# MITIBMxGraph/SALIENT_plusplus

Hardware: AMD Instinct MI355X
Metric: sampled_edges_per_sec (higher is better)
Workload: dtype int64/fp16-copy

## Files before the change

### include/spp.h

```cpp
#ifndef SPP_H
#define SPP_H

#include <stddef.h>
#include <stdint.h>

#ifdef __cplusplus
extern "C" {
#endif

#define SPP_ABI_VERSION 6
#define SPP_MAX_HOPS 8
#define SPP_MAX_PARTS 64

typedef int spp_status;
enum {
  SPP_OK = 0,
  SPP_ERR_INVALID = -1,
  SPP_ERR_HIP = -2,
  SPP_ERR_CAPACITY = -3,
  SPP_ERR_STATE = -4
};

int spp_abi_version(void);
const char* spp_last_error(void);
// ... 37 lines not shown
  int64_t cache_map_len;
} spp_partition_cfg;

typedef struct spp_sampler_opts {
  int32_t col32;
  int32_t deg_tags;
  int32_t row_stubs;
  int32_t rng_arena;
  int64_t rng_arena_mb;
  int32_t fuse_scatter;
  int32_t flag_tiled;
  int32_t rows_coalesced;
  int32_t dedup_preread;
  int64_t fuse_max_edges;
  int64_t initial_edge_cap;
  int64_t reserved[4];
} spp_sampler_opts;

typedef struct spp_sampler_cfg {
  const int64_t* rowptr_dev;
  const int64_t* col_dev;
  int64_t num_nodes;
  int64_t nnz;
  int32_t num_hops;
  int64_t sizes[SPP_MAX_HOPS];
  int64_t max_batch;
  int32_t num_slots;
  int32_t device;
  int32_t replace;
  spp_partition_cfg part;
  int64_t graph_generation;
// ... 5 lines not shown
  int32_t deg_tags;
  int32_t row_stubs;
  int32_t rng_arena;
  int32_t idbits, tag_cap;
  int32_t num_hops;
  int32_t dedup_buckets_log2;
  int32_t dedup_table_slots;
  int32_t generic[SPP_MAX_HOPS];
  int32_t fused_pick[SPP_MAX_HOPS];
  int32_t flag_tiled[SPP_MAX_HOPS];
  int32_t rows_coalesced[SPP_MAX_HOPS];
  int32_t bucket_log2[SPP_MAX_HOPS];
  double col32_ms, row_stubs_ms, rng_arena_ms;
  int64_t col32_bytes, row_stubs_bytes, rng_arena_bytes;
  int64_t rng_arena_batches;
} spp_sampler_info;

typedef struct spp_mfg_counts {
  int64_t num_nodes;
  int64_t num_seeds;
  int32_t num_hops;
  int64_t T[SPP_MAX_HOPS];
  int64_t S[SPP_MAX_HOPS];
  int64_t E[SPP_MAX_HOPS];
  int64_t draws;
  int64_t part_counts[SPP_MAX_PARTS + 2];
} spp_mfg_counts;

typedef struct spp_mfg_out {
  int64_t* n_id;
// ... 846 lines not shown
```

### salient_plusplus_amd/_native.py

```python
import ctypes as C
import os

_HERE = os.path.dirname(os.path.abspath(__file__))
LIB_PATH = os.path.join(_HERE, "libspp_hip.so")

SPP_MAX_HOPS = 8
SPP_MAX_PARTS = 64

p = C.c_void_p
i32 = C.c_int32
i64 = C.c_int64
u32 = C.c_uint32


class PartitionCfg(C.Structure):
    _fields_ = [("num_parts", i32), ("rank", i32), ("offsets", i64 * (SPP_MAX_PARTS + 1)),
                ("use_cache", i32), ("cache_map_dev", p), ("cache_map_len", i64)]


class SamplerOpts(C.Structure):
    _fields_ = [("col32", i32), ("deg_tags", i32), ("row_stubs", i32), ("rng_arena", i32), ("rng_arena_mb", i64),
                ("fuse_scatter", i32), ("flag_tiled", i32), ("rows_coalesced", i32), ("dedup_preread", i32),
                ("fuse_max_edges", i64), ("initial_edge_cap", i64), ("reserved", i64 * 4)]


class SamplerCfg(C.Structure):
    _fields_ = [("rowptr_dev", p), ("col_dev", p), ("num_nodes", i64), ("nnz", i64),
                ("num_hops", i32), ("sizes", i64 * SPP_MAX_HOPS), ("max_batch", i64),
                ("num_slots", i32), ("device", i32), ("replace", i32), ("part", PartitionCfg),
                ("graph_generation", i64), ("opts", SamplerOpts)]


class SamplerInfo(C.Structure):
    _fields_ = [("col32", i32), ("deg_tags", i32), ("row_stubs", i32), ("rng_arena", i32), ("idbits", i32),
                ("tag_cap", i32), ("num_hops", i32), ("dedup_buckets_log2", i32), ("dedup_table_slots", i32),
                ("generic", i32 * SPP_MAX_HOPS), ("fused_pick", i32 * SPP_MAX_HOPS), ("flag_tiled", i32 * SPP_MAX_HOPS),
                ("rows_coalesced", i32 * SPP_MAX_HOPS), ("bucket_log2", i32 * SPP_MAX_HOPS),
                ("col32_ms", C.c_double), ("row_stubs_ms", C.c_double), ("rng_arena_ms", C.c_double),
                ("col32_bytes", i64), ("row_stubs_bytes", i64), ("rng_arena_bytes", i64), ("rng_arena_batches", i64)]


class MfgCounts(C.Structure):
    _fields_ = [("num_nodes", i64), ("num_seeds", i64), ("num_hops", i32),
                ("T", i64 * SPP_MAX_HOPS), ("S", i64 * SPP_MAX_HOPS), ("E", i64 * SPP_MAX_HOPS),
                ("draws", i64), ("part_counts", i64 * (SPP_MAX_PARTS + 2))]


class MfgOut(C.Structure):
    _fields_ = [("n_id", p), ("rowptr", p * SPP_MAX_HOPS), ("col", p * SPP_MAX_HOPS),
                ("parts", p), ("cached", p), ("perm", p), ("row_addr", p), ("x_remote", p)]


SPP_ELEM_F32, SPP_ELEM_F16, SPP_ELEM_BF16 = 0, 1, 2
SPP_BN_ACT_NONE, SPP_BN_ACT_RELU, SPP_BN_ACT_LEAKY_RELU = 0, 1, 2
# ... 383 lines not shown
```

### salient_plusplus_amd/csrc/sampler.hip

```cpp
#include "spp_internal.h"

#include <hipcub/hipcub.hpp>

#include <algorithm>
#include <chrono>
#include <cstdlib>
#include <cstring>
#include <vector>

#include <map>
#include <memory>
#include <mutex>
#include <tuple>

#include "fp8_body.hip.h"
#include "gather_body.hip.h"
#include "partition_common.hip.h"

#ifndef SPP_TILE_NT
#define SPP_TILE_NT 1024
#endif
#include "mt19937.hip.h"
#include "sampler_internal.h"

// ... 1984 lines not shown
  void* cub_tmp = nullptr;
  size_t cub_tmp_bytes = 0;
};

struct ResolvedOpts {
  int col32 = 1;
  int deg_tags = 1;
  int row_stubs = -1;
  int rng_arena = -1;
  int64_t rng_arena_words = 0;
  int fuse = 1;
  int64_t fuse_max_edges = 262144;
  bool flag_tiled = true, rows_coalesced = true, dedup_preread = false;
};

struct HopPlan {
  bool self_prefix = false;
  bool fused = false;
  bool flag_tiled = false;
  bool rows_coal = false;
  unsigned row_lds = 0;
  unsigned lds_fused = 0;
  int64_t tile_cap = 0;
};

struct spp_sampler {
  spp_sampler_cfg cfg{};
  ResolvedOpts opt{};
  HopPlan plan[SPP_MAX_HOPS];
  int rng_arena_decision = -1;
  double col32_ms = 0, stubs_ms = 0;
  hipEvent_t arena_t0 = nullptr, arena_t1 = nullptr;
  double rng_arena_ms = 0;
  bool arena_timed = false;
  int64_t tcap[SPP_MAX_HOPS + 1];
  int64_t ecap[SPP_MAX_HOPS];
  int64_t dcap = 0;
  bool generic[SPP_MAX_HOPS];
  bool any_generic = false;
  DedupGeom geom{};
  int cb_log2[SPP_MAX_HOPS];
  int lds_log2 = 12;
  int64_t bytes = 0;
  std::vector<SlotHost> slots;
// ... 61 lines not shown
  SPP_REQUIRE(cfg->max_batch > 0 && cfg->num_slots > 0, "spp_sampler_create: max_batch and num_slots must be > 0");
  const spp_partition_cfg& pc = cfg->part;
  SPP_REQUIRE(pc.num_parts >= 0 && pc.num_parts <= SPP_MAX_PARTS, "spp_sampler_create: num_parts %d not in [0,%d]",
              pc.num_parts, SPP_MAX_PARTS);
  if (pc.num_parts > 0) {
    SPP_REQUIRE(pc.rank >= 0 && pc.rank < pc.num_parts, "spp_sampler_create: rank %d out of [0,%d)", pc.rank,
                pc.num_parts);
    SPP_REQUIRE(!pc.use_cache || (pc.cache_map_dev && pc.cache_map_len > 0),
                "spp_sampler_create: use_cache without a cache map");
    for (int m = 0; m < pc.num_parts; ++m)
      SPP_REQUIRE(pc.offsets[m] <= pc.offsets[m + 1], "spp_sampler_create: partition offsets must be non-decreasing");
    SPP_REQUIRE(pc.offsets[0] <= 0 && pc.offsets[pc.num_parts] >= cfg->num_nodes,
                "spp_sampler_create: partition offsets [%lld,%lld) do not cover the %lld nodes",
                (long long)pc.offsets[0], (long long)pc.offsets[pc.num_parts], (long long)cfg->num_nodes);
  }
  int ndev = spp_device_count();
  SPP_REQUIRE(ndev > 0, "spp_sampler_create: no HIP device available (the on-GPU sampler has no CPU fallback)");
  SPP_HIP_TRY(hipSetDevice(cfg->device));

  auto* s = new spp_sampler();
  s->cfg = *cfg;
  if (const char* e = getenv("SPP_XCD_AFFINITY")) s->xcd_affinity = atoi(e) != 0;
  {
    const spp_sampler_opts& o = cfg->opts;
    auto env_int = [](const char* name, long long dflt) -> long long {
      const char* e = getenv(name);
      return e && *e ? atoll(e) : dflt;
    };
    auto sw = [&](int32_t field, const char* name, int dflt) -> int {
      if (field) return field > 0 ? 1 : 0;
// ... 6 lines not shown
    else {
      const long long m = env_int("SPP_ROW_STUBS", -1);
      r.row_stubs = m < 0 ? -1 : (m > 0 ? 1 : 0);
    }
    const bool env_budget = getenv("SPP_RNG_ARENA_MB") != nullptr;
    const long long mb = o.rng_arena_mb > 0 ? o.rng_arena_mb : env_int("SPP_RNG_ARENA_MB", 16384);
    r.rng_arena_words = (mb < 0 ? 0 : mb) * (int64_t)(1 << 20) / 4;
    if (o.rng_arena) r.rng_arena = o.rng_arena > 0 ? 1 : 0;
    else r.rng_arena = (o.rng_arena_mb > 0 || env_budget) ? 1 : -1;
    if (o.fuse_scatter) r.fuse = o.fuse_scatter < 0 ? 0 : std::min(o.fuse_scatter, 2);
    else r.fuse = (int)std::max<long long>(0, std::min<long long>(2, env_int("SPP_FUSE_SCATTER", 1)));
    r.fuse_max_edges = o.fuse_max_edges > 0 ? o.fuse_max_edges : env_int("SPP_FUSE_MAX_EDGES", 262144);
    r.flag_tiled = sw(o.flag_tiled, "SPP_FLAG_TILED", 1) != 0;
    r.rows_coalesced = sw(o.rows_coalesced, "SPP_ROWS_COALESCED", 1) != 0;
    r.dedup_preread = sw(o.dedup_preread, "SPP_DEDUP_PREREAD", 0) != 0;
  }
  const int H = cfg->num_hops;
  const int64_t node_bound = cfg->num_nodes + cfg->max_batch;
  s->tcap[0] = cfg->max_batch;
  int64_t etmp = 1;
  for (int h = 0; h < H; ++h) {
    const int64_t f = cfg->sizes[h];
    s->generic[h] = (f < 0 || f > kFastMaxFanout);
    s->any_generic |= s->generic[h];
    if (f >= 0) {
      s->ecap[h] = s->tcap[h] * f;
      s->tcap[h + 1] = std::min(s->tcap[h] * (1 + f), node_bound);
      s->dcap += f * s->tcap[h];
    } else {
      s->ecap[h] = cfg->opts.initial_edge_cap > 0 ? cfg->opts.initial_edge_cap
// ... 18 lines not shown
  s->geom.nb_log2 = nb_log2;
  s->geom.nb = 1 << nb_log2;
  const int64_t per_bucket = (ucap + s->geom.nb - 1) / s->geom.nb;
  s->geom.kcap = (int32_t)std::min<int64_t>(per_bucket + per_bucket / 2 + 256, 0x7fffffff);
  s->lds_log2 = per_bucket > 6144 ? 14 : (per_bucket > 1536 ? 13 : (per_bucket > 820 ? 12 : 11));
  for (int h = 0; h < H; ++h) {
    int c = std::max(0, nb_log2 - kMaxFineLog2);
    while (c < nb_log2 && (s->tcap[h + 1] >> c) > bucket_nodes) ++c;
    s->cb_log2[h] = c;
  }
  const int nb = s->geom.nb;
  int64_t tmax = 0;
  for (int h = 0; h < H; ++h) tmax = std::max(tmax, s->tcap[h]);
  const int64_t nblk_max = std::max(ceil_div(tmax, kNT), ceil_div(etmp, kNT)) + 1;
  const int nslots = cfg->num_slots;
  if (pc.num_parts > 0) {
    s->part.P = pc.num_parts;
    s->part.rank = pc.rank;
    s->part.use_cache = pc.use_cache ? 1 : 0;
    s->part.cache_map = pc.cache_map_dev;
    s->part.cache_len = pc.cache_map_len;
    s->part.off.n = pc.num_parts + 1;
    for (int m = 0; m <= pc.num_parts; ++m) s->part.off.v[m] = pc.offsets[m];
    s->part.nblk_cap = (int32_t)ceil_div(ucap, kNT);
  }

  s->slots.resize(nslots);
  spp_status rc = SPP_OK;
  void* v = nullptr;
  rc = dev_alloc(s, &v, sizeof(SlotPtrs) * (size_t)nslots);
// ... 43 lines not shown
      A(p.parts, int32_t, ucap);
      A(p.pcached, int32_t, ucap);
      A(p.pperm, int32_t, ucap);
      A(p.psrc, int2, ucap);
      A(p.pbucket, uint8_t, ucap);
      A(p.pblk, int32_t, (int64_t)(s->part.P + 1) * s->part.nblk_cap);
    }
#undef A
    p.kcount = s->counts + (size_t)i * (size_t)s->counts_per_slot;
    p.bfill = p.kcount + nb;
    p.ctr = p.bfill + nb;
    p.ovfc = p.ctr + 1;
    p.st = s->d_states + i;
    sl.host_state = s->h_states + i;
    if (rc == SPP_OK) {
      sl.etmp_cap = etmp;
      hipError_t e = hipMalloc((void**)&p.cval, sizeof(int32_t) * (size_t)etmp);
      const size_t n_bucketed = (size_t)(region_for(etmp) + etmp);
      if (e == hipSuccess) e = hipMalloc((void**)&p.bpairs, sizeof(unsigned long long) * n_bucketed);
      if (e == hipSuccess) e = hipMalloc((void**)&p.evals, sizeof(uint32_t) * (size_t)etmp);
      if (e == hipSuccess) e = hipMalloc((void**)&p.inv, sizeof(uint32_t) * (size_t)etmp);
      if (e == hipSuccess) e = hipMalloc((void**)&p.tidx, sizeof(uint16_t) * (size_t)etmp);
      if (e == hipSuccess) e = hipMalloc((void**)&p.res, sizeof(uint32_t) * n_bucketed);
      if (e == hipSuccess) e = hipMalloc((void**)&p.fwords, rank_bytes(etmp));
      if (e == hipSuccess) p.fsum = reinterpret_cast<int32_t*>(reinterpret_cast<char*>(p.fwords) + rank_off_fsum(etmp));
      if (e != hipSuccess) {
        set_error("spp_sampler_create: hipMalloc of edge scratch failed: %s", hipGetErrorString(e));
        rc = SPP_ERR_HIP;
      }
      s->bytes += 14 * etmp + 12 * (int64_t)n_bucketed + (int64_t)rank_bytes(etmp);
    }
    if (rc == SPP_OK && (hipEventCreateWithFlags(&sl.done, hipEventDisableTiming) != hipSuccess ||
                         hipEventCreateWithFlags(&sl.exported, hipEventDisableTiming) != hipSuccess)) {
      set_error("spp_sampler_create: hipEventCreate failed");
      rc = SPP_ERR_HIP;
    }
  }
  if (rc == SPP_OK && cfg->nnz > 0 && s->opt.col32) {
    std::lock_guard<std::mutex> lk(g_col32_mu);
    int idbits = 1;
    while (idbits < 32 && ((int64_t)1 << idbits) < cfg->num_nodes) ++idbits;
    const bool want_tags = s->opt.deg_tags && idbits <= 29;
    const auto key = std::make_tuple((const void*)cfg->col_dev, cfg->nnz, (int)cfg->device, cfg->graph_generation,
                                     want_tags ? 1 : 0);
    std::shared_ptr<Col32> c = g_col32[key].lock();
// ... 168 lines not shown
  s->workers[1].reset();
  (void)hipSetDevice(s->cfg.device);
  (void)hipDeviceSynchronize();
  for (auto& sl : s->slots) {
    if (sl.done) (void)hipEventDestroy(sl.done);
    if (sl.exported) (void)hipEventDestroy(sl.exported);
    if (sl.p.cval) (void)hipFree(sl.p.cval);
    if (sl.p.bpairs) (void)hipFree(sl.p.bpairs);
    if (sl.p.evals) (void)hipFree(sl.p.evals);
    if (sl.p.inv) (void)hipFree(sl.p.inv);
    if (sl.p.tidx) (void)hipFree(sl.p.tidx);
    if (sl.p.res) (void)hipFree(sl.p.res);
    if (sl.p.fwords) (void)hipFree(sl.p.fwords);
    if (sl.cub_tmp) (void)hipFree(sl.cub_tmp);
  }
  if (s->rng_arena) (void)hipFree(s->rng_arena);
  if (s->rng_arena_seeds_dev) (void)hipFree(s->rng_arena_seeds_dev);
  if (s->rng_arena_ready) (void)hipEventDestroy(s->rng_arena_ready);
  if (s->arena_t0) (void)hipEventDestroy(s->arena_t0);
  if (s->arena_t1) (void)hipEventDestroy(s->arena_t1);
  if (s->inputs_ready) (void)hipEventDestroy(s->inputs_ready);
  if (s->cache_bits_ready) (void)hipEventDestroy(s->cache_bits_ready);
  if (s->cache_bits) (void)hipFree(s->cache_bits);
  if (s->h_states) (void)hipHostFree(s->h_states);
  if (s->deliver_stream) (void)hipStreamDestroy(s->deliver_stream);
  for (auto st : s->work_streams)
    if (st) (void)hipStreamDestroy(st);
  if (s->comm_stream) (void)hipStreamDestroy(s->comm_stream);
  for (auto& d : s->dargs_host)
    if (d) (void)hipHostFree(d);
// ... 46 lines not shown
  if (s->arena_timed) {
    (void)hipSetDevice(s->cfg.device);
    float ms = 0.f;
    if (hipEventSynchronize(s->arena_t1) == hipSuccess && hipEventElapsedTime(&ms, s->arena_t0, s->arena_t1) == hipSuccess)
      s->rng_arena_ms = ms;
    (void)hipGetLastError();
    s->arena_timed = false;
  }
  out->col32_ms = s->col32_ms;
  out->row_stubs_ms = s->stubs_ms;
  out->rng_arena_ms = s->rng_arena_ms;
  out->col32_bytes = s->col32 ? (int64_t)sizeof(int32_t) * (s->cfg.nnz + 16) : 0;
  out->row_stubs_bytes = s->stubs ? (int64_t)sizeof(int32_t) * kStubInts * s->cfg.num_nodes : 0;
  out->rng_arena_bytes = 4 * s->rng_arena_words;
  out->rng_arena_batches = (int64_t)s->rng_arena_seeds.size();
  return SPP_OK;
}

static spp_status grow_edge_scratch(spp_sampler* s, int slot, int h, int64_t need, hipStream_t st) {
  SlotHost& sl = s->slots[(size_t)slot];
  bool changed = false;
  if (need > sl.etmp_cap) {
    int64_t cap = std::max(need, sl.etmp_cap * 2);
    RankWord* old_fwords = sl.p.fwords;
    int32_t* old_fsum = sl.p.fsum;
    const int64_t old_cap = sl.etmp_cap;
    (void)hipFree(sl.p.cval); (void)hipFree(sl.p.bpairs); (void)hipFree(sl.p.evals);
    (void)hipFree(sl.p.inv); (void)hipFree(sl.p.res); (void)hipFree(sl.p.tidx);
    sl.p.tidx = nullptr;
    sl.p.cval = nullptr; sl.p.bpairs = nullptr; sl.p.evals = nullptr; sl.p.fwords = nullptr;
// ... 17 lines not shown
  }
  if (need > sl.ecap_dyn[h]) {
    int64_t cap = std::max(need, sl.ecap_dyn[h] * 2);
    void* v = nullptr;
    SPP_HIP_TRY(hipMalloc(&v, sizeof(int32_t) * (size_t)cap));
    s->allocs.push_back(v);
    sl.p.out_col[h] = static_cast<int32_t*>(v);
    s->bytes += 4 * cap;
    sl.ecap_dyn[h] = cap;
    changed = true;
  }
  if (changed) SPP_TRY(upload_slot(s, slot, st));
  return SPP_OK;
}

namespace spp {

int sampler_max_group(const spp_sampler* s) { return s->any_generic ? 1 : kMaxGroup; }

hipStream_t sampler_work_stream(spp_sampler* s, int i) {
  static const int n_streams = [] {
    const char* e = getenv("SPP_WORK_STREAMS");
    const int v = e ? atoi(e) : 2;
    return v < 1 ? 1 : (v > kMaxWorkStreams ? kMaxWorkStreams : v);
  }();
  hipStream_t& st = s->work_streams[i % n_streams];
  if (!st && create_data_stream(&st, true) != hipSuccess) st = nullptr;
  return st;
}

// ... 105 lines not shown
  SlotHost& lead = s->slots[(size_t)first_slot];
  const int32_t interleave = s->xcd_affinity ? 1 : 0;
  auto GG = [&](unsigned gx) { return GroupGrid{(int32_t)first_slot, (int32_t)n, gx, interleave}; };

  static const struct Dup { int count, pick, flag, rows; } dup = [] {
    Dup d{1, 1, 1, 1};
    if (const char* e = getenv("SPP_WHATIF_DUP")) {
      if (strstr(e, "count")) d.count = 2;
      if (strstr(e, "pick")) d.pick = 2;
      if (strstr(e, "flag")) d.flag = 2;
      if (strstr(e, "rows")) d.rows = 2;
    }
    return d;
  }();
  const DedupGeom geom = s->geom;
  const int prof = prof_begin(SPP_PROF_CHAIN, st, n);
  SPP_HIP_TRY(hipMemsetAsync(lead.p.kcount, 0, sizeof(int32_t) * (size_t)s->counts_per_slot * (size_t)n, st));
  const unsigned gseed = (unsigned)ceil_div(max_seeds, kNT);
  ga.grid = GG(gseed);
  hipLaunchKernelGGL(k_seed_init, dim3(gseed * gy), dim3(kNT), 0, st, s->d_slots, ga, geom, rowptr, stubs,
                     (int32_t)s->cfg.sizes[0], replace, s->tag_cap);
  const uint32_t idmask = s->idmask;
  const uint32_t pick_mask = s->use_tags ? 0xffffffffu : idmask;
  const int32_t row_idbits = s->use_tags ? s->idbits : 32;
  for (int h = 0; h < H; ++h) {
    const int32_t f = (int32_t)s->cfg.sizes[h];
    const unsigned gt = (unsigned)std::max<int64_t>(1, ceil_div(s->tcap[h], kNT));
    const HopPlan& pl = s->plan[h];
    const unsigned row_lds = pl.row_lds;
    for (int rep = 0; h > 0 && rep < dup.count; ++rep) {
      const unsigned gc = (gt + kNT / kWave - 1) / (kNT / kWave);
      hipLaunchKernelGGL(k_hop_count, dim3((gc) * gy), dim3(kNT), 0, st, s->d_slots, GG(gc), rowptr, stubs, s->use_tags ? 1 : 0, h, f, replace, (int32_t)s->tcap[h]);
    }
    const int32_t ecap_dev =
        s->generic[h] ? 0x7fffffff : (int32_t)std::min<int64_t>(lead.ecap_dyn[h], 0x7fffffff);
    const int32_t self_prefix = pl.self_prefix ? 1 : 0;
    if (!self_prefix)
      hipLaunchKernelGGL(k_hop_scan, dim3((1) * gy), dim3(kScanNT), 0, st, s->d_slots, GG(1), h, f, ecap_dev, s->dcap);
    const FuseArgs fa_plain{};
    unsigned ge;
    for (int rep = 0; !s->generic[h] && rep < dup.pick - 1; ++rep)
      if (col32 && stubs && s->use_tags)
        hipLaunchKernelGGL((k_hop_pick<false, int32_t, true, true>), dim3((gt) * gy), dim3(kNT), row_lds, st, s->d_slots, GG(gt),
                           col32, stubs, h, f, replace, self_prefix, ecap_dev, s->dcap, (int32_t)s->tcap[h], pick_mask, fa_plain);
    const int32_t cb = s->cb_log2[h];
    const unsigned nbk = 1u << cb;
    const int64_t pcap = std::max<int64_t>(1, s->generic[h] ? 0 : s->ecap[h]);
    const bool fused = pl.fused;
    const int64_t tile_cap = pl.tile_cap;
    const unsigned lds_fused = pl.lds_fused;
    if (!s->generic[h]) {
      if (fused) {
        FuseArgs fa{cb, bucket_cap(pcap, nbk), (int32_t)region_for(lead.etmp_cap), idmask, (int32_t)(row_lds / sizeof(int32_t)), (int32_t)tile_cap};
        const unsigned lds = lds_fused;
        hipLaunchKernelGGL((k_hop_pick<false, int32_t, true, true, true>), dim3((gt) * gy), dim3(kNT), lds, st, s->d_slots, GG(gt),
                           col32, stubs, h, f, replace, self_prefix, ecap_dev, s->dcap, (int32_t)s->tcap[h], pick_mask, fa);
      } else if (col32 && stubs && s->use_tags)
        hipLaunchKernelGGL((k_hop_pick<false, int32_t, true, true>), dim3((gt) * gy), dim3(kNT), row_lds, st, s->d_slots, GG(gt),
                           col32, stubs, h, f, replace, self_prefix, ecap_dev, s->dcap, (int32_t)s->tcap[h], pick_mask, fa_plain);
      else if (col32 && stubs)
        hipLaunchKernelGGL((k_hop_pick<false, int32_t, true>), dim3((gt) * gy), dim3(kNT), row_lds, st, s->d_slots, GG(gt),
                           col32, stubs, h, f, replace, self_prefix, ecap_dev, s->dcap, (int32_t)s->tcap[h], pick_mask, fa_plain);
      else if (col32)
        hipLaunchKernelGGL((k_hop_pick<false, int32_t, false>), dim3((gt) * gy), dim3(kNT), row_lds, st, s->d_slots, GG(gt),
                           col32, stubs, h, f, replace, self_prefix, ecap_dev, s->dcap, (int32_t)s->tcap[h], pick_mask, fa_plain);
      else if (stubs)
        hipLaunchKernelGGL((k_hop_pick<false, int64_t, true>), dim3((gt) * gy), dim3(kNT), row_lds, st, s->d_slots, GG(gt),
                           col, stubs, h, f, replace, self_prefix, ecap_dev, s->dcap, (int32_t)s->tcap[h], pick_mask, fa_plain);
      else
        hipLaunchKernelGGL((k_hop_pick<false, int64_t, false>), dim3((gt) * gy), dim3(kNT), row_lds, st, s->d_slots, GG(gt),
                           col, stubs, h, f, replace, self_prefix, ecap_dev, s->dcap, (int32_t)s->tcap[h], pick_mask, fa_plain);
      ge = (unsigned)std::max<int64_t>(1, ceil_div(s->ecap[h], kNT));
    } else {
      SPP_HIP_TRY(hipMemcpyAsync(lead.host_state, lead.p.st, sizeof(SlotState), hipMemcpyDeviceToHost, st));
      SPP_HIP_TRY(hipStreamSynchronize(st));
      const int64_t E = lead.host_state->E[h];
      if (lead.host_state->error) break;
      SPP_TRY(grow_edge_scratch(s, first_slot, h, E, st));
      ge = (unsigned)std::max<int64_t>(1, ceil_div(E, kNT));
      hipLaunchKernelGGL((k_hop_pick<true, int64_t, false>), dim3((gt) * gy), dim3(kNT), sizeof(int32_t) * kNT, st, s->d_slots,
                         GG(gt), col, stubs, h, f, replace, 0, ecap_dev, s->dcap, (int32_t)s->tcap[h], pick_mask, fa_plain);
      if (col32)
        hipLaunchKernelGGL(k_hop_expand_generic<int32_t>, dim3((ge) * gy), dim3(kNT), 0, st, s->d_slots, GG(ge), col32,
                           h, f, replace, idmask);
      else
        hipLaunchKernelGGL(k_hop_expand_generic<int64_t>, dim3((ge) * gy), dim3(kNT), 0, st, s->d_slots, GG(ge), col,
                           h, f, replace, idmask);
    }
    const int32_t region = (int32_t)region_for(lead.etmp_cap);
    const bool dedup_preread = s->opt.dedup_preread;
    const int32_t last = ((h == H - 1) ? 1 : 0) | (!dedup_preread ? 2 : 0);
    const int32_t hop_word = h | (s->cb_log2[h] << 8) | (last << 16);
    const int64_t pcap_h = s->generic[h] ? std::max<int64_t>(1, lead.host_state->E[h]) : pcap;
    const unsigned gsc = (unsigned)std::max<int64_t>(1, ceil_div((int64_t)ge * kNT, kScatterTile));
    const unsigned sc_lds = (unsigned)(sizeof(int32_t) * 2 * nbk + (sizeof(uint32_t) + sizeof(uint16_t)) * kScatterTile);
    const int32_t bcap = bucket_cap(pcap_h, nbk);
    const bool flag_tiled = pl.flag_tiled;
    if (!fused)
      hipLaunchKernelGGL(k_bucket_scatter, dim3((gsc) * gy), dim3(kTileNT), sc_lds, st, s->d_slots, GG(gsc), h, cb, bcap, region, pcap_h, idmask,
                         flag_tiled ? 1 : 0);
    static const unsigned dedup_pad = [] { const char* e = getenv("SPP_WHATIF_DEDUP_LDS_PAD"); return e ? (unsigned)atoi(e) : 0u; }();
    const unsigned dpad = (h == H - 1) ? dedup_pad : 0u;
    static const bool dedup_flat_on = [] { const char* e = getenv("SPP_DEDUP_FLAT"); return !e || atoi(e) != 0; }();
    const bool flat = dedup_flat_on && (geom.nb_log2 - cb) > 2;
    if (s->lds_log2 == 11 && flat)
      hipLaunchKernelGGL((k_bucket_dedup<2048, true>), dim3((nbk) * gy), dim3(kNT), dpad, st, s->d_slots, GG(nbk), hop_word, geom, bcap, region);
    else if (s->lds_log2 == 12 && flat)
      hipLaunchKernelGGL((k_bucket_dedup<SPP_DEDUP_SLOTS12, true>), dim3((nbk) * gy), dim3(kNT), dpad, st, s->d_slots, GG(nbk), hop_word, geom, bcap, region);
    else if (s->lds_log2 == 11)
      hipLaunchKernelGGL(k_bucket_dedup<2048>, dim3((nbk) * gy), dim3(kNT), dpad, st, s->d_slots, GG(nbk), hop_word, geom, bcap, region);
    else if (s->lds_log2 == 12)
      hipLaunchKernelGGL(k_bucket_dedup<SPP_DEDUP_SLOTS12>, dim3((nbk) * gy), dim3(kNT), dpad, st, s->d_slots, GG(nbk), hop_word, geom, bcap, region);
    else if (s->lds_log2 == 13)
      hipLaunchKernelGGL(k_bucket_dedup<8192>, dim3((nbk) * gy), dim3(kNT), 0, st, s->d_slots, GG(nbk), hop_word, geom, bcap, region);
    else
      hipLaunchKernelGGL(k_bucket_dedup<16384>, dim3((nbk) * gy), dim3(kNT), 0, st, s->d_slots, GG(nbk), hop_word, geom, bcap, region);
    const unsigned gflag = (unsigned)std::max<int64_t>(1, ceil_div((int64_t)ge * kNT, kFlagSpan));
    for (int rep = 0; rep < dup.flag; ++rep) {
      if (flag_tiled)
        hipLaunchKernelGGL(k_hop_flag_tiled, dim3((gsc) * gy), dim3(kFlagNT), 0, st, s->d_slots, GG(gsc), h, f,
                           (int32_t)s->tcap[H], pcap_h);
      else
        hipLaunchKernelGGL(k_hop_flag, dim3((gflag) * gy), dim3(kFlagNT), 0, st, s->d_slots, GG(gflag), h, f,
                           (int32_t)s->tcap[H], pcap_h);
    }
    if (!s->generic[h]) {
      const int32_t run_cap = (int32_t)(kNT * std::max<int32_t>(1, std::min<int32_t>(f, kFastMaxFanout)));
      for (int rep = 0; rep < dup.rows; ++rep) {
        if (pl.rows_coal)
          hipLaunchKernelGGL(k_hop_rows_coalesced, dim3((gt) * gy), dim3(kNT), (unsigned)(8 * run_cap), st, s->d_slots, GG(gt), h,
                             idmask, row_idbits, (int32_t)s->tcap[h], pcap_h, run_cap);
        else
          hipLaunchKernelGGL(k_hop_rows, dim3((gt) * gy), dim3(kNT), row_lds, st, s->d_slots, GG(gt), h, idmask, row_idbits,
                             (int32_t)s->tcap[h], pcap_h);
      }
    } else {
      const int64_t E = lead.host_state->E[h];
      const int32_t T = lead.host_state->cnt[h];
      if (E > 0) {
        hipLaunchKernelGGL(k_hop_lids_generic, dim3((ge) * gy), dim3(kNT), 0, st, s->d_slots, GG(ge), h);
        size_t need = 0;
        SPP_HIP_TRY(hipcub::DeviceSegmentedRadixSort::SortKeys(nullptr, need, lead.p.cval, lead.p.out_col[h], (int)E, T,
                                                               lead.p.out_rowptr[h], lead.p.out_rowptr[h] + 1, 0, 32,
                                                               st));
        if (need > lead.cub_tmp_bytes) {
          SPP_HIP_TRY(hipStreamSynchronize(st));
          if (lead.cub_tmp) (void)hipFree(lead.cub_tmp);
          lead.cub_tmp = nullptr;
          SPP_HIP_TRY(hipMalloc(&lead.cub_tmp, need));
          lead.cub_tmp_bytes = need;
        }
        size_t have = lead.cub_tmp_bytes;
        SPP_HIP_TRY(hipcub::DeviceSegmentedRadixSort::SortKeys(lead.cub_tmp, have, lead.p.cval, lead.p.out_col[h],
                                                               (int)E, T, lead.p.out_rowptr[h],
                                                               lead.p.out_rowptr[h] + 1, 0, 32, st));
      }
    }
  }
  if (s->part.P > 0) {
    const unsigned gu = (unsigned)std::max<int64_t>(1, ceil_div(s->tcap[H], kPartSpan));
    hipLaunchKernelGGL(k_gpart_hist, dim3((gu) * gy), dim3(kNT), 0, st, s->d_slots, GG(gu), H, s->part, (int32_t)s->tcap[H]);
    hipLaunchKernelGGL(k_gpart_scan, dim3((1) * gy), dim3(kScanNT), 0, st, s->d_slots, GG(1), H, s->part);
    hipLaunchKernelGGL(k_gpart_scatter, dim3((gu) * gy), dim3(kNT), 0, st, s->d_slots, GG(gu), H, s->part, (int32_t)s->tcap[H]);
  }
  prof_end(SPP_PROF_CHAIN, prof, st);
  SPP_HIP_TRY(hipGetLastError());
  SPP_HIP_TRY(hipMemcpyAsync(lead.host_state, lead.p.st, sizeof(SlotState) * (size_t)n, hipMemcpyDeviceToHost, st));
  SPP_HIP_TRY(hipEventRecord(lead.done, st));
  for (int i = 0; i < n; ++i) {
    SlotHost& sl = s->slots[(size_t)(first_slot + i)];
    sl.wait_on = lead.done;
    sl.sampled = true;
// ... 462 lines not shown
```

### salient_plusplus_amd/fast_sampler/__init__.py

```python
import collections
import ctypes as C
import datetime
import math
import os
import threading
from typing import List, Optional, Sequence

import torch

from .. import _native as nat
from ..fp8 import Fp8Features

__all__ = ["Config", "Session", "ProtoDistributedBatch", "RangePartitionBook", "Cache", "sample_adj",
           "multilayer_sample", "full_sample", "to_row_major", "serial_index", "NativeComm", "native_comm",
           "set_native_comm", "async_errors", "set_sampler_options", "sampler_options", "sampler_info", "TableRows", "RowRefs", "Fp8Features", "fp8_gather_rows", "resident_graph", "resident_partition",
           "P2PPeers", "set_p2p_peers", "p2p_open_peers"]

_MAX_SLOTS = int(os.environ.get("SPP_MAX_SLOTS", "64"))
_MAX_SLOTS_DIST = int(os.environ.get("SPP_MAX_SLOTS_DIST", "64"))
_LOOKAHEAD_GROUPS = max(1, int(os.environ.get("SPP_LOOKAHEAD_GROUPS", "2")))


def _lib():
    L = nat.load()
# ... 539 lines not shown
        rank, world = dist.get_rank(group), dist.get_world_size(group)
        buf = torch.zeros(nat.SPP_COMM_ID_BYTES, dtype=torch.uint8)
        if rank == 0:
            nat.check(L.spp_comm_unique_id(C.c_void_p(buf.data_ptr())))
        buf = buf.to(dev)
        dist.broadcast(buf, src=dist.get_global_rank(group, 0) if group is not None else 0, group=group)
        token = buf.cpu().contiguous()
        h = C.c_void_p()
        nat.check(L.spp_comm_create(C.c_void_p(token.data_ptr()), rank, world, dev.index, C.byref(h)))
        comm = NativeComm(h, rank, world)
        _comm_auto[key] = comm
        return comm


_OPT_FIELDS = ("col32", "deg_tags", "row_stubs", "rng_arena", "rng_arena_mb", "fuse_scatter", "flag_tiled",
               "rows_coalesced", "dedup_preread", "fuse_max_edges", "initial_edge_cap")
_sampler_opts = {}


def set_sampler_options(**kw):
    for k in kw:
        if k not in _OPT_FIELDS:
            raise RuntimeError(f"unknown sampler option {k!r} (known: {', '.join(_OPT_FIELDS)})")
    _sampler_opts.clear()
    for k, v in kw.items():
        if isinstance(v, bool):
            v = 1 if v else -1
        if int(v) != 0:
            _sampler_opts[k] = int(v)


# ... 1076 lines not shown
```

Measured before the change: 8.664 billion.

## Run last hop in sub-batches over a shared per-stream edge scratch pool

Per-slot edge scratch is now sized for the largest non-final hop. The last hop, which has the largest edge count, runs in sub-groups of up to last_hop_sub slots that reuse a per-stream pool of full-size scratch sets. This shrinks the workspace footprint and working set, which should improve cache residency and allow more slots. The cost is that the last hop's kernels are launched several times instead of once, and pool creation can force a device synchronize when the stream LRU evicts.

```diff
diff --git a/include/spp.h b/include/spp.h
--- a/include/spp.h
+++ b/include/spp.h
@@ -75,7 +75,8 @@
   int32_t dedup_preread;
   int64_t fuse_max_edges;
   int64_t initial_edge_cap;
-  int64_t reserved[4];
+  int64_t last_hop_sub;
+  int64_t reserved[3];
 } spp_sampler_opts;
 
 typedef struct spp_sampler_cfg {
@@ -111,6 +112,9 @@
   double col32_ms, row_stubs_ms, rng_arena_ms;
   int64_t col32_bytes, row_stubs_bytes, rng_arena_bytes;
   int64_t rng_arena_batches;
+  int32_t last_hop_sub;
+  int32_t last_hop_pool_sets;
+  int64_t workspace_bytes;
 } spp_sampler_info;
 
 typedef struct spp_mfg_counts {
diff --git a/salient_plusplus_amd/_native.py b/salient_plusplus_amd/_native.py
--- a/salient_plusplus_amd/_native.py
+++ b/salient_plusplus_amd/_native.py
@@ -21,7 +21,8 @@
 class SamplerOpts(C.Structure):
     _fields_ = [("col32", i32), ("deg_tags", i32), ("row_stubs", i32), ("rng_arena", i32), ("rng_arena_mb", i64),
                 ("fuse_scatter", i32), ("flag_tiled", i32), ("rows_coalesced", i32), ("dedup_preread", i32),
-                ("fuse_max_edges", i64), ("initial_edge_cap", i64), ("reserved", i64 * 4)]
+                ("fuse_max_edges", i64), ("initial_edge_cap", i64), ("last_hop_sub", i64),
+                ("reserved", i64 * 3)]
 
 
 class SamplerCfg(C.Structure):
@@ -37,7 +38,8 @@
                 ("generic", i32 * SPP_MAX_HOPS), ("fused_pick", i32 * SPP_MAX_HOPS), ("flag_tiled", i32 * SPP_MAX_HOPS),
                 ("rows_coalesced", i32 * SPP_MAX_HOPS), ("bucket_log2", i32 * SPP_MAX_HOPS),
                 ("col32_ms", C.c_double), ("row_stubs_ms", C.c_double), ("rng_arena_ms", C.c_double),
-                ("col32_bytes", i64), ("row_stubs_bytes", i64), ("rng_arena_bytes", i64), ("rng_arena_batches", i64)]
+                ("col32_bytes", i64), ("row_stubs_bytes", i64), ("rng_arena_bytes", i64), ("rng_arena_batches", i64),
+                ("last_hop_sub", i32), ("last_hop_pool_sets", i32), ("workspace_bytes", i64)]
 
 
 class MfgCounts(C.Structure):
diff --git a/salient_plusplus_amd/csrc/sampler.hip b/salient_plusplus_amd/csrc/sampler.hip
--- a/salient_plusplus_amd/csrc/sampler.hip
+++ b/salient_plusplus_amd/csrc/sampler.hip
@@ -2022,6 +2022,18 @@
   bool flag_tiled = true, rows_coalesced = true, dedup_preread = false;
 };
 
+#ifndef SPP_LAST_HOP_SUB
+#define SPP_LAST_HOP_SUB 16
+#endif
+
+struct LastPool {
+  hipStream_t stream = nullptr;
+  SlotPtrs* d_tab = nullptr;
+  void* block = nullptr;
+  uint64_t stamp = 0;
+};
+constexpr int kMaxPools = 8;
+
 struct HopPlan {
   bool self_prefix = false;
   bool fused = false;
@@ -2036,6 +2048,12 @@
   spp_sampler_cfg cfg{};
   ResolvedOpts opt{};
   HopPlan plan[SPP_MAX_HOPS];
+  int last_sub = kMaxGroup;
+  int pool_n = 0;
+  int64_t etmp_big = 0;
+  std::vector<LastPool> pools;
+  std::mutex pool_mu;
+  uint64_t pool_clock = 0;
   int rng_arena_decision = -1;
   double col32_ms = 0, stubs_ms = 0;
   hipEvent_t arena_t0 = nullptr, arena_t1 = nullptr;
@@ -2127,6 +2145,9 @@
                 "spp_sampler_create: partition offsets [%lld,%lld) do not cover the %lld nodes",
                 (long long)pc.offsets[0], (long long)pc.offsets[pc.num_parts], (long long)cfg->num_nodes);
   }
+  SPP_REQUIRE(cfg->opts.last_hop_sub >= 0 && cfg->opts.last_hop_sub <= kMaxGroup,
+              "spp_sampler_create: last_hop_sub %lld not in [0,%d] (0 = the library's default)",
+              (long long)cfg->opts.last_hop_sub, kMaxGroup);
   int ndev = spp_device_count();
   SPP_REQUIRE(ndev > 0, "spp_sampler_create: no HIP device available (the on-GPU sampler has no CPU fallback)");
   SPP_HIP_TRY(hipSetDevice(cfg->device));
@@ -2163,6 +2184,7 @@
     r.flag_tiled = sw(o.flag_tiled, "SPP_FLAG_TILED", 1) != 0;
     r.rows_coalesced = sw(o.rows_coalesced, "SPP_ROWS_COALESCED", 1) != 0;
     r.dedup_preread = sw(o.dedup_preread, "SPP_DEDUP_PREREAD", 0) != 0;
+    s->last_sub = o.last_hop_sub > 0 ? (int)o.last_hop_sub : std::min<int>(SPP_LAST_HOP_SUB, kMaxGroup);
   }
   const int H = cfg->num_hops;
   const int64_t node_bound = cfg->num_nodes + cfg->max_batch;
@@ -2211,6 +2233,10 @@
   for (int h = 0; h < H; ++h) tmax = std::max(tmax, s->tcap[h]);
   const int64_t nblk_max = std::max(ceil_div(tmax, kNT), ceil_div(etmp, kNT)) + 1;
   const int nslots = cfg->num_slots;
+  int64_t etmp_small = 1;
+  for (int h = 0; h + 1 < H; ++h) etmp_small = std::max(etmp_small, s->ecap[h]);
+  s->etmp_big = etmp;
+  if (!s->any_generic && nslots > 2 * s->last_sub && etmp_small < etmp) s->pool_n = s->last_sub;
   if (pc.num_parts > 0) {
     s->part.P = pc.num_parts;
     s->part.rank = pc.rank;
@@ -2284,13 +2310,14 @@
     p.st = s->d_states + i;
     sl.host_state = s->h_states + i;
     if (rc == SPP_OK) {
-      sl.etmp_cap = etmp;
-      hipError_t e = hipMalloc((void**)&p.cval, sizeof(int32_t) * (size_t)etmp);
-      const size_t n_bucketed = (size_t)(region_for(etmp) + etmp);
+      const int64_t escr = s->pool_n > 0 ? etmp_small : etmp;
+      sl.etmp_cap = escr;
+      hipError_t e = hipMalloc((void**)&p.cval, sizeof(int32_t) * (size_t)escr);
+      const size_t n_bucketed = (size_t)(region_for(escr) + escr);
       if (e == hipSuccess) e = hipMalloc((void**)&p.bpairs, sizeof(unsigned long long) * n_bucketed);
-      if (e == hipSuccess) e = hipMalloc((void**)&p.evals, sizeof(uint32_t) * (size_t)etmp);
-      if (e == hipSuccess) e = hipMalloc((void**)&p.inv, sizeof(uint32_t) * (size_t)etmp);
-      if (e == hipSuccess) e = hipMalloc((void**)&p.tidx, sizeof(uint16_t) * (size_t)etmp);
+      if (e == hipSuccess) e = hipMalloc((void**)&p.evals, sizeof(uint32_t) * (size_t)escr);
+      if (e == hipSuccess) e = hipMalloc((void**)&p.inv, sizeof(uint32_t) * (size_t)escr);
+      if (e == hipSuccess) e = hipMalloc((void**)&p.tidx, sizeof(uint16_t) * (size_t)escr);
       if (e == hipSuccess) e = hipMalloc((void**)&p.res, sizeof(uint32_t) * n_bucketed);
       if (e == hipSuccess) e = hipMalloc((void**)&p.fwords, rank_bytes(etmp));
       if (e == hipSuccess) p.fsum = reinterpret_cast<int32_t*>(reinterpret_cast<char*>(p.fwords) + rank_off_fsum(etmp));
@@ -2298,7 +2325,7 @@
         set_error("spp_sampler_create: hipMalloc of edge scratch failed: %s", hipGetErrorString(e));
         rc = SPP_ERR_HIP;
       }
-      s->bytes += 14 * etmp + 12 * (int64_t)n_bucketed + (int64_t)rank_bytes(etmp);
+      s->bytes += 14 * escr + 12 * (int64_t)n_bucketed + (int64_t)rank_bytes(etmp);
     }
     if (rc == SPP_OK && (hipEventCreateWithFlags(&sl.done, hipEventDisableTiming) != hipSuccess ||
                          hipEventCreateWithFlags(&sl.exported, hipEventDisableTiming) != hipSuccess)) {
@@ -2497,6 +2524,10 @@
     if (sl.p.fwords) (void)hipFree(sl.p.fwords);
     if (sl.cub_tmp) (void)hipFree(sl.cub_tmp);
   }
+  for (auto& pl : s->pools) {
+    if (pl.block) (void)hipFree(pl.block);
+    if (pl.d_tab) (void)hipFree(pl.d_tab);
+  }
   if (s->rng_arena) (void)hipFree(s->rng_arena);
   if (s->rng_arena_seeds_dev) (void)hipFree(s->rng_arena_seeds_dev);
   if (s->rng_arena_ready) (void)hipEventDestroy(s->rng_arena_ready);
@@ -2573,6 +2604,9 @@
   out->row_stubs_bytes = s->stubs ? (int64_t)sizeof(int32_t) * kStubInts * s->cfg.num_nodes : 0;
   out->rng_arena_bytes = 4 * s->rng_arena_words;
   out->rng_arena_batches = (int64_t)s->rng_arena_seeds.size();
+  out->last_hop_sub = s->last_sub;
+  out->last_hop_pool_sets = s->pool_n;
+  out->workspace_bytes = s->bytes;
   return SPP_OK;
 }
 
@@ -2620,6 +2654,65 @@
   return SPP_OK;
 }
 
+static spp_status last_pool_for(spp_sampler* s, hipStream_t st, LastPool** out) {
+  std::lock_guard<std::mutex> lk(s->pool_mu);
+  for (LastPool& p : s->pools)
+    if (p.stream == st) {
+      p.stamp = ++s->pool_clock;
+      *out = &p;
+      return SPP_OK;
+    }
+  if ((int)s->pools.size() >= kMaxPools) {
+    SPP_HIP_TRY(hipDeviceSynchronize());
+    LastPool* lru = &s->pools[0];
+    for (LastPool& p : s->pools)
+      if (p.stamp < lru->stamp) lru = &p;
+    lru->stream = st;
+    lru->stamp = ++s->pool_clock;
+    *out = lru;
+    return SPP_OK;
+  }
+  const int64_t cap = s->etmp_big;
+  const size_t n_bucketed = (size_t)(region_for(cap) + cap);
+  auto up = [](size_t b) { return (b + 255) / 256 * 256; };
+  const size_t o_evals = up(4 * (size_t)cap), o_inv = o_evals + up(4 * (size_t)cap), o_res = o_inv + up(4 * (size_t)cap);
+  const size_t o_bpairs = o_res + up(4 * n_bucketed), o_tidx = o_bpairs + up(8 * n_bucketed);
+  const size_t set_bytes = o_tidx + up(2 * (size_t)cap);
+  const size_t nslots = s->slots.size();
+  LastPool p;
+  p.stream = st;
+  SPP_HIP_TRY(hipMalloc(&p.block, set_bytes * (size_t)s->pool_n));
+  if (hipMalloc((void**)&p.d_tab, sizeof(SlotPtrs) * nslots) != hipSuccess) {
+    (void)hipFree(p.block);
+    set_error("spp_sampler: hipMalloc of the last hop's slot table failed");
+    return SPP_ERR_HIP;
+  }
+  std::vector<SlotPtrs> tab(nslots);
+  for (size_t i = 0; i < nslots; ++i) {
+    SlotPtrs& t = tab[i] = s->slots[i].p;
+    char* base = static_cast<char*>(p.block) + set_bytes * (i % (size_t)s->pool_n);
+    t.cval = reinterpret_cast<int32_t*>(base);
+    t.evals = reinterpret_cast<uint32_t*>(base + o_evals);
+    t.inv = reinterpret_cast<uint32_t*>(base + o_inv);
+    t.res = reinterpret_cast<uint32_t*>(base + o_res);
+    t.bpairs = reinterpret_cast<unsigned long long*>(base + o_bpairs);
+    t.tidx = reinterpret_cast<uint16_t*>(base + o_tidx);
+  }
+  const hipError_t e = hipMemcpy(p.d_tab, tab.data(), sizeof(SlotPtrs) * nslots, hipMemcpyHostToDevice);
+  if (e != hipSuccess) {
+    (void)hipFree(p.block);
+    (void)hipFree(p.d_tab);
+    set_error("spp_sampler: upload of the last hop's slot table failed: %s", hipGetErrorString(e));
+    return SPP_ERR_HIP;
+  }
+  s->bytes += (int64_t)(set_bytes * (size_t)s->pool_n + sizeof(SlotPtrs) * nslots);
+  p.stamp = ++s->pool_clock;
+  s->pools.reserve(kMaxPools);
+  s->pools.push_back(p);
+  *out = &s->pools.back();
+  return SPP_OK;
+}
+
 namespace spp {
 
 int sampler_max_group(const spp_sampler* s) { return s->any_generic ? 1 : kMaxGroup; }
@@ -2755,6 +2848,8 @@
     return d;
   }();
   const DedupGeom geom = s->geom;
+  LastPool* pool = nullptr;
+  if (s->pool_n > 0) SPP_TRY(last_pool_for(s, st, &pool));
   const int prof = prof_begin(SPP_PROF_CHAIN, st, n);
   SPP_HIP_TRY(hipMemsetAsync(lead.p.kcount, 0, sizeof(int32_t) * (size_t)s->counts_per_slot * (size_t)n, st));
   const unsigned gseed = (unsigned)ceil_div(max_seeds, kNT);
@@ -2778,11 +2873,20 @@
     const int32_t self_prefix = pl.self_prefix ? 1 : 0;
     if (!self_prefix)
       hipLaunchKernelGGL(k_hop_scan, dim3((1) * gy), dim3(kScanNT), 0, st, s->d_slots, GG(1), h, f, ecap_dev, s->dcap);
+    const bool last_hop = h == H - 1;
+    const int run_len = (last_hop && !s->generic[h]) ? std::min(n, s->last_sub) : n;
+    const SlotPtrs* const d_slots = (last_hop && pool) ? pool->d_tab : s->d_slots;
+    const bool pooled_last = last_hop && pool;
+    bool failed = false;
+    for (int b0 = 0; b0 < n && !failed; b0 += run_len) {
+    const int nr = std::min(run_len, n - b0);
+    const unsigned gy = (unsigned)nr;
+    auto GG = [&](unsigned gx) { return GroupGrid{(int32_t)(first_slot + b0), (int32_t)nr, gx, interleave}; };
     const FuseArgs fa_plain{};
     unsigned ge;
     for (int rep = 0; !s->generic[h] && rep < dup.pick - 1; ++rep)
       if (col32 && stubs && s->use_tags)
-        hipLaunchKernelGGL((k_hop_pick<false, int32_t, true, true>), dim3((gt) * gy), dim3(kNT), row_lds, st, s->d_slots, GG(gt),
+        hipLaunchKernelGGL((k_hop_pick<false, int32_t, true, true>), dim3((gt) * gy), dim3(kNT), row_lds, st, d_slots, GG(gt),
                            col32, stubs, h, f, replace, self_prefix, ecap_dev, s->dcap, (int32_t)s->tcap[h], pick_mask, fa_plain);
     const int32_t cb = s->cb_log2[h];
     const unsigned nbk = 1u << cb;
@@ -2792,43 +2896,46 @@
     const unsigned lds_fused = pl.lds_fused;
     if (!s->generic[h]) {
       if (fused) {
-        FuseArgs fa{cb, bucket_cap(pcap, nbk), (int32_t)region_for(lead.etmp_cap), idmask, (int32_t)(row_lds / sizeof(int32_t)), (int32_t)tile_cap};
+        FuseArgs fa{cb, bucket_cap(pcap, nbk), (int32_t)region_for(pooled_last ? s->etmp_big : lead.etmp_cap), idmask, (int32_t)(row_lds / sizeof(int32_t)), (int32_t)tile_cap};
         const unsigned lds = lds_fused;
-        hipLaunchKernelGGL((k_hop_pick<false, int32_t, true, true, true>), dim3((gt) * gy), dim3(kNT), lds, st, s->d_slots, GG(gt),
+        hipLaunchKernelGGL((k_hop_pick<false, int32_t, true, true, true>), dim3((gt) * gy), dim3(kNT), lds, st, d_slots, GG(gt),
                            col32, stubs, h, f, replace, self_prefix, ecap_dev, s->dcap, (int32_t)s->tcap[h], pick_mask, fa);
       } else if (col32 && stubs && s->use_tags)
-        hipLaunchKernelGGL((k_hop_pick<false, int32_t, true, true>), dim3((gt) * gy), dim3(kNT), row_lds, st, s->d_slots, GG(gt),
+        hipLaunchKernelGGL((k_hop_pick<false, int32_t, true, true>), dim3((gt) * gy), dim3(kNT), row_lds, st, d_slots, GG(gt),
                            col32, stubs, h, f, replace, self_prefix, ecap_dev, s->dcap, (int32_t)s->tcap[h], pick_mask, fa_plain);
       else if (col32 && stubs)
-        hipLaunchKernelGGL((k_hop_pick<false, int32_t, true>), dim3((gt) * gy), dim3(kNT), row_lds, st, s->d_slots, GG(gt),
+        hipLaunchKernelGGL((k_hop_pick<false, int32_t, true>), dim3((gt) * gy), dim3(kNT), row_lds, st, d_slots, GG(gt),
                            col32, stubs, h, f, replace, self_prefix, ecap_dev, s->dcap, (int32_t)s->tcap[h], pick_mask, fa_plain);
       else if (col32)
-        hipLaunchKernelGGL((k_hop_pick<false, int32_t, false>), dim3((gt) * gy), dim3(kNT), row_lds, st, s->d_slots, GG(gt),
+        hipLaunchKernelGGL((k_hop_pick<false, int32_t, false>), dim3((gt) * gy), dim3(kNT), row_lds, st, d_slots, GG(gt),
                            col32, stubs, h, f, replace, self_prefix, ecap_dev, s->dcap, (int32_t)s->tcap[h], pick_mask, fa_plain);
       else if (stubs)
-        hipLaunchKernelGGL((k_hop_pick<false, int64_t, true>), dim3((gt) * gy), dim3(kNT), row_lds, st, s->d_slots, GG(gt),
+        hipLaunchKernelGGL((k_hop_pick<false, int64_t, true>), dim3((gt) * gy), dim3(kNT), row_lds, st, d_slots, GG(gt),
                            col, stubs, h, f, replace, self_prefix, ecap_dev, s->dcap, (int32_t)s->tcap[h], pick_mask, fa_plain);
       else
-        hipLaunchKernelGGL((k_hop_pick<false, int64_t, false>), dim3((gt) * gy), dim3(kNT), row_lds, st, s->d_slots, GG(gt),
+        hipLaunchKernelGGL((k_hop_pick<false, int64_t, false>), dim3((gt) * gy), dim3(kNT), row_lds, st, d_slots, GG(gt),
                            col, stubs, h, f, replace, self_prefix, ecap_dev, s->dcap, (int32_t)s->tcap[h], pick_mask, fa_plain);
       ge = (unsigned)std::max<int64_t>(1, ceil_div(s->ecap[h], kNT));
     } else {
       SPP_HIP_TRY(hipMemcpyAsync(lead.host_state, lead.p.st, sizeof(SlotState), hipMemcpyDeviceToHost, st));
       SPP_HIP_TRY(hipStreamSynchronize(st));
       const int64_t E = lead.host_state->E[h];
-      if (lead.host_state->error) break;
+      if (lead.host_state->error) {
+        failed = true;
+        break;
+      }
       SPP_TRY(grow_edge_scratch(s, first_slot, h, E, st));
       ge = (unsigned)std::max<int64_t>(1, ceil_div(E, kNT));
-      hipLaunchKernelGGL((k_hop_pick<true, int64_t, false>), dim3((gt) * gy), dim3(kNT), sizeof(int32_t) * kNT, st, s->d_slots,
+      hipLaunchKernelGGL((k_hop_pick<true, int64_t, false>), dim3((gt) * gy), dim3(kNT), sizeof(int32_t) * kNT, st, d_slots,
                          GG(gt), col, stubs, h, f, replace, 0, ecap_dev, s->dcap, (int32_t)s->tcap[h], pick_mask, fa_plain);
       if (col32)
-        hipLaunchKernelGGL(k_hop_expand_generic<int32_t>, dim3((ge) * gy), dim3(kNT), 0, st, s->d_slots, GG(ge), col32,
+        hipLaunchKernelGGL(k_hop_expand_generic<int32_t>, dim3((ge) * gy), dim3(kNT), 0, st, d_slots, GG(ge), col32,
                            h, f, replace, idmask);
       else
-        hipLaunchKernelGGL(k_hop_expand_generic<int64_t>, dim3((ge) * gy), dim3(kNT), 0, st, s->d_slots, GG(ge), col,
+        hipLaunchKernelGGL(k_hop_expand_generic<int64_t>, dim3((ge) * gy), dim3(kNT), 0, st, d_slots, GG(ge), col,
                            h, f, replace, idmask);
     }
-    const int32_t region = (int32_t)region_for(lead.etmp_cap);
+    const int32_t region = (int32_t)region_for(pooled_last ? s->etmp_big : lead.etmp_cap);
     const bool dedup_preread = s->opt.dedup_preread;
     const int32_t last = ((h == H - 1) ? 1 : 0) | (!dedup_preread ? 2 : 0);
     const int32_t hop_word = h | (s->cb_log2[h] << 8) | (last << 16);
@@ -2838,48 +2945,48 @@
     const int32_t bcap = bucket_cap(pcap_h, nbk);
     const bool flag_tiled = pl.flag_tiled;
     if (!fused)
-      hipLaunchKernelGGL(k_bucket_scatter, dim3((gsc) * gy), dim3(kTileNT), sc_lds, st, s->d_slots, GG(gsc), h, cb, bcap, region, pcap_h, idmask,
+      hipLaunchKernelGGL(k_bucket_scatter, dim3((gsc) * gy), dim3(kTileNT), sc_lds, st, d_slots, GG(gsc), h, cb, bcap, region, pcap_h, idmask,
                          flag_tiled ? 1 : 0);
     static const unsigned dedup_pad = [] { const char* e = getenv("SPP_WHATIF_DEDUP_LDS_PAD"); return e ? (unsigned)atoi(e) : 0u; }();
     const unsigned dpad = (h == H - 1) ? dedup_pad : 0u;
     static const bool dedup_flat_on = [] { const char* e = getenv("SPP_DEDUP_FLAT"); return !e || atoi(e) != 0; }();
     const bool flat = dedup_flat_on && (geom.nb_log2 - cb) > 2;
     if (s->lds_log2 == 11 && flat)
-      hipLaunchKernelGGL((k_bucket_dedup<2048, true>), dim3((nbk) * gy), dim3(kNT), dpad, st, s->d_slots, GG(nbk), hop_word, geom, bcap, region);
+      hipLaunchKernelGGL((k_bucket_dedup<2048, true>), dim3((nbk) * gy), dim3(kNT), dpad, st, d_slots, GG(nbk), hop_word, geom, bcap, region);
     else if (s->lds_log2 == 12 && flat)
-      hipLaunchKernelGGL((k_bucket_dedup<SPP_DEDUP_SLOTS12, true>), dim3((nbk) * gy), dim3(kNT), dpad, st, s->d_slots, GG(nbk), hop_word, geom, bcap, region);
+      hipLaunchKernelGGL((k_bucket_dedup<SPP_DEDUP_SLOTS12, true>), dim3((nbk) * gy), dim3(kNT), dpad, st, d_slots, GG(nbk), hop_word, geom, bcap, region);
     else if (s->lds_log2 == 11)
-      hipLaunchKernelGGL(k_bucket_dedup<2048>, dim3((nbk) * gy), dim3(kNT), dpad, st, s->d_slots, GG(nbk), hop_word, geom, bcap, region);
+      hipLaunchKernelGGL(k_bucket_dedup<2048>, dim3((nbk) * gy), dim3(kNT), dpad, st, d_slots, GG(nbk), hop_word, geom, bcap, region);
     else if (s->lds_log2 == 12)
-      hipLaunchKernelGGL(k_bucket_dedup<SPP_DEDUP_SLOTS12>, dim3((nbk) * gy), dim3(kNT), dpad, st, s->d_slots, GG(nbk), hop_word, geom, bcap, region);
+      hipLaunchKernelGGL(k_bucket_dedup<SPP_DEDUP_SLOTS12>, dim3((nbk) * gy), dim3(kNT), dpad, st, d_slots, GG(nbk), hop_word, geom, bcap, region);
     else if (s->lds_log2 == 13)
-      hipLaunchKernelGGL(k_bucket_dedup<8192>, dim3((nbk) * gy), dim3(kNT), 0, st, s->d_slots, GG(nbk), hop_word, geom, bcap, region);
+      hipLaunchKernelGGL(k_bucket_dedup<8192>, dim3((nbk) * gy), dim3(kNT), 0, st, d_slots, GG(nbk), hop_word, geom, bcap, region);
     else
-      hipLaunchKernelGGL(k_bucket_dedup<16384>, dim3((nbk) * gy), dim3(kNT), 0, st, s->d_slots, GG(nbk), hop_word, geom, bcap, region);
+      hipLaunchKernelGGL(k_bucket_dedup<16384>, dim3((nbk) * gy), dim3(kNT), 0, st, d_slots, GG(nbk), hop_word, geom, bcap, region);
     const unsigned gflag = (unsigned)std::max<int64_t>(1, ceil_div((int64_t)ge * kNT, kFlagSpan));
     for (int rep = 0; rep < dup.flag; ++rep) {
       if (flag_tiled)
-        hipLaunchKernelGGL(k_hop_flag_tiled, dim3((gsc) * gy), dim3(kFlagNT), 0, st, s->d_slots, GG(gsc), h, f,
+        hipLaunchKernelGGL(k_hop_flag_tiled, dim3((gsc) * gy), dim3(kFlagNT), 0, st, d_slots, GG(gsc), h, f,
                            (int32_t)s->tcap[H], pcap_h);
       else
-        hipLaunchKernelGGL(k_hop_flag, dim3((gflag) * gy), dim3(kFlagNT), 0, st, s->d_slots, GG(gflag), h, f,
+        hipLaunchKernelGGL(k_hop_flag, dim3((gflag) * gy), dim3(kFlagNT), 0, st, d_slots, GG(gflag), h, f,
                            (int32_t)s->tcap[H], pcap_h);
     }
     if (!s->generic[h]) {
       const int32_t run_cap = (int32_t)(kNT * std::max<int32_t>(1, std::min<int32_t>(f, kFastMaxFanout)));
       for (int rep = 0; rep < dup.rows; ++rep) {
         if (pl.rows_coal)
-          hipLaunchKernelGGL(k_hop_rows_coalesced, dim3((gt) * gy), dim3(kNT), (unsigned)(8 * run_cap), st, s->d_slots, GG(gt), h,
+          hipLaunchKernelGGL(k_hop_rows_coalesced, dim3((gt) * gy), dim3(kNT), (unsigned)(8 * run_cap), st, d_slots, GG(gt), h,
                              idmask, row_idbits, (int32_t)s->tcap[h], pcap_h, run_cap);
         else
-          hipLaunchKernelGGL(k_hop_rows, dim3((gt) * gy), dim3(kNT), row_lds, st, s->d_slots, GG(gt), h, idmask, row_idbits,
+          hipLaunchKernelGGL(k_hop_rows, dim3((gt) * gy), dim3(kNT), row_lds, st, d_slots, GG(gt), h, idmask, row_idbits,
                              (int32_t)s->tcap[h], pcap_h);
       }
     } else {
       const int64_t E = lead.host_state->E[h];
       const int32_t T = lead.host_state->cnt[h];
       if (E > 0) {
-        hipLaunchKernelGGL(k_hop_lids_generic, dim3((ge) * gy), dim3(kNT), 0, st, s->d_slots, GG(ge), h);
+        hipLaunchKernelGGL(k_hop_lids_generic, dim3((ge) * gy), dim3(kNT), 0, st, d_slots, GG(ge), h);
         size_t need = 0;
         SPP_HIP_TRY(hipcub::DeviceSegmentedRadixSort::SortKeys(nullptr, need, lead.p.cval, lead.p.out_col[h], (int)E, T,
                                                                lead.p.out_rowptr[h], lead.p.out_rowptr[h] + 1, 0, 32,
@@ -2897,6 +3004,8 @@
                                                                lead.p.out_rowptr[h] + 1, 0, 32, st));
       }
     }
+    }
+    if (failed) break;
   }
   if (s->part.P > 0) {
     const unsigned gu = (unsigned)std::max<int64_t>(1, ceil_div(s->tcap[H], kPartSpan));
diff --git a/salient_plusplus_amd/fast_sampler/__init__.py b/salient_plusplus_amd/fast_sampler/__init__.py
--- a/salient_plusplus_amd/fast_sampler/__init__.py
+++ b/salient_plusplus_amd/fast_sampler/__init__.py
@@ -577,7 +577,7 @@
 
 
 _OPT_FIELDS = ("col32", "deg_tags", "row_stubs", "rng_arena", "rng_arena_mb", "fuse_scatter", "flag_tiled",
-               "rows_coalesced", "dedup_preread", "fuse_max_edges", "initial_edge_cap")
+               "rows_coalesced", "dedup_preread", "fuse_max_edges", "initial_edge_cap", "last_hop_sub")
 _sampler_opts = {}
 
 
```

Result: slower. 8.486 billion (-2.1%).
